# Ivordir/YALPS

Measured on AMD Instinct MI355X. Metric: fp64 pivots/sec on dense m x n tableau, higher is better.
Workload: dtype f64

## Files before the change

### yalps_amd/build.py

```python
import os
import re
import shutil
import subprocess

HERE = os.path.dirname(os.path.abspath(__file__))
ROOT = os.path.dirname(HERE)
LIB = os.path.join(HERE, "libyalps_hip.so")
LIB_STAMPS = os.path.join(HERE, "libyalps_hip_stamps.so")
LINK_LIBS = []
CSRC = os.path.join(HERE, "csrc")
HIP_SRC = os.path.join(CSRC, "yalps_hip.hip")
HIP_UNITS = [HIP_SRC] + [os.path.join(CSRC, f) for f in sorted(os.listdir(CSRC)) if f.startswith("persistent_") and f.endswith(".hip")]
HIP_DEPS = [os.path.join(CSRC, f) for f in sorted(os.listdir(CSRC)) if f.endswith((".cuh", ".inc", ".h")) and not f.startswith(("lp_batch", "lp_dense", "lp_variants", "lp_sens", "lp_warm", "milp_node", "milp_tree", "milp_dense", "wg_queue"))]
LIB_LPBATCH = os.path.join(HERE, "libyalps_lpbatch.so")
LPBATCH_SRC = os.path.join(CSRC, "lp_batch.hip")
QUEUE_DEPS = [os.path.join(CSRC, f) for f in ("wg_queue.cuh", "wg_queue_host.inc", "wg_simplex.cuh", "common.cuh")]
LPBATCH_DEPS = [os.path.join(CSRC, f) for f in ("lp_batch_kernel.cuh", "lp_batch_host.inc", "lp_batch_lib.inc")] + QUEUE_DEPS
LPBATCH_HEADER = os.path.join(ROOT, "include", "yalps_lpbatch.h")
LIB_MILPBATCH = os.path.join(HERE, "libyalps_milpbatch.so")
MILPBATCH_SRC = os.path.join(CSRC, "milp_batch.hip")
MILPBATCH_DEPS = LPBATCH_DEPS + [os.path.join(CSRC, f) for f in ("milp_node_kernel.cuh", "milp_search.inc")] + [LPBATCH_HEADER]
MILPBATCH_HEADER = os.path.join(ROOT, "include", "yalps_milpbatch.h")
LIB_LPVAR = os.path.join(HERE, "libyalps_lpvar.so")
LPVAR_SRC = os.path.join(CSRC, "lp_variants.hip")
LPVAR_DEPS = [os.path.join(CSRC, "lp_variants_kernel.cuh")] + QUEUE_DEPS
LPVAR_HEADER = os.path.join(ROOT, "include", "yalps_lpvar.h")
LIB_LPSENS = os.path.join(HERE, "libyalps_lpsens.so")
LPSENS_SRC = os.path.join(CSRC, "lp_sens.hip")
LPSENS_DEPS = [os.path.join(CSRC, "lp_sens_kernel.cuh")] + LPBATCH_DEPS
LPSENS_HEADER = os.path.join(ROOT, "include", "yalps_lpsens.h")
LIB_LPWARM = os.path.join(HERE, "libyalps_lpwarm.so")
LPWARM_SRC = os.path.join(CSRC, "lp_warm.hip")
LPWARM_DEPS = [os.path.join(CSRC, "lp_warm_kernel.cuh")] + LPBATCH_DEPS + [LPBATCH_HEADER]
LPWARM_HEADER = os.path.join(ROOT, "include", "yalps_lpwarm.h")
LIB_MILPTREE = os.path.join(HERE, "libyalps_milptree.so")
MILPTREE_SRC = os.path.join(CSRC, "milp_tree.hip")
MILPTREE_DEPS = LPBATCH_DEPS + [os.path.join(CSRC, f) for f in ("milp_tree_kernel.cuh", "milp_tree_rules.cuh", "milp_tree_host.inc")] + [LPBATCH_HEADER]
MILPTREE_HEADER = os.path.join(ROOT, "include", "yalps_milptree.h")
LIB_LPDENSE = os.path.join(HERE, "libyalps_lpdense.so")
LPDENSE_SRC = os.path.join(CSRC, "lp_dense.hip")
LPDENSE_DEPS = [os.path.join(CSRC, "lp_dense_kernel.cuh")] + QUEUE_DEPS
LIB_LPDENSE_BOUNDS = os.path.join(HERE, "libyalps_lpdense_bounds.so")
LPDENSE_BOUNDS_SRC = os.path.join(CSRC, "lp_dense_bounds.hip")
LPDENSE_HEADER = os.path.join(ROOT, "include", "yalps_lpdense.h")
LIB_LPDENSE_FREE = os.path.join(HERE, "libyalps_lpdense_free.so")
LPDENSE_FREE_SRC = os.path.join(CSRC, "lp_dense_free.hip")
LIB_MILPDENSE = os.path.join(HERE, "libyalps_milpdense.so")
MILPDENSE_SRC = os.path.join(CSRC, "milp_dense.hip")
MILPDENSE_DEPS = [os.path.join(CSRC, f) for f in ("milp_dense_kernel.cuh", "milp_tree_kernel.cuh", "milp_tree_rules.cuh", "milp_tree_host.inc",
                                                  "lp_batch_kernel.cuh", "milp_dense_bounds_kernel.cuh", "milp_dense_free_kernel.cuh")] + QUEUE_DEPS
MILPDENSE_HEADER = os.path.join(ROOT, "include", "yalps_milpdense.h")
LIB_MILPDENSE_BOUNDS = os.path.join(HERE, "libyalps_milpdense_bounds.so")
MILPDENSE_BOUNDS_SRC = os.path.join(CSRC, "milp_dense_bounds.hip")
MILPDENSE_BOUNDS_DEPS = [os.path.join(CSRC, f) for f in ("milp_dense_bounds_kernel.cuh", "milp_dense_kernel.cuh", "milp_tree_rules.cuh")] + QUEUE_DEPS
LIB_MILPDENSE_FREE = os.path.join(HERE, "libyalps_milpdense_free.so")
MILPDENSE_FREE_SRC = os.path.join(CSRC, "milp_dense_free.hip")
MILPDENSE_FREE_DEPS = [os.path.join(CSRC, "milp_dense_free_kernel.cuh")] + MILPDENSE_BOUNDS_DEPS
OBJ_DIR = os.path.join(HERE, "build")
HEADER = os.path.join(ROOT, "include", "yalps_hip.h")
NAPI_SRC = os.path.join(HERE, "napi", "yalps_napi.cc")
NAPI_OUT = os.path.join(HERE, "napi", "yalps_napi.node")

HIPCC_FLAGS = ["--offload-arch=gfx950", "-O3", "-std=c++17", "-ffp-contract=off", "-fPIC"]


def _stale(out, *srcs):
    return not os.path.exists(out) or any(os.path.getmtime(out) < os.path.getmtime(s) for s in srcs if os.path.exists(s))


def kernel_metadata(lib=LIB):
    import re
    import tempfile
    llvm = "/opt/rocm/lib/llvm/bin"
    with tempfile.TemporaryDirectory() as tmp:
        fat, co = os.path.join(tmp, "fat.bin"), os.path.join(tmp, "dev.co")
        subprocess.run([f"{llvm}/llvm-objcopy", "-O", "binary", "--only-section=.hip_fatbin", lib, fat], check=True)
        magic = b"__CLANG_OFFLOAD_BUNDLE__"
        blob = open(fat, "rb").read()
        starts = [i for i in range(len(blob)) if blob.startswith(magic, i)]
        if not starts:
            raise RuntimeError("no offload bundle in .hip_fatbin of %s" % lib)
        notes = ""
        for k, lo in enumerate(starts):
            part = os.path.join(tmp, "part%d.bin" % k)
            with open(part, "wb") as f:
                f.write(blob[lo:starts[k + 1] if k + 1 < len(starts) else len(blob)])
            subprocess.run([f"{llvm}/clang-offload-bundler", "--unbundle", "--type=o", f"--input={part}",
                            "--targets=hipv4-amdgcn-amd-amdhsa--gfx950", f"--output={co}"], check=True)
            notes += subprocess.run([f"{llvm}/llvm-readelf", "--notes", co], check=True, capture_output=True, text=True).stdout
    kernels, cur = {}, {}
    for line in notes.splitlines():
        m = re.match(r"\s*(?:- )?\.(\w+):\s+(\S+)\s*$", line)
        if not m:
            continue
        key, val = m.groups()
        if key == "agpr_count" and line.lstrip().startswith("- "):
            cur = {}
        cur[key] = val
        if key == "name" and val.startswith("_Z"):
            kernels[val] = cur
    return kernels


NO_SCRATCH = ("lp_sens", "lp_dense", "milp_dense_root_kernel", "milp_dense_solution_kernel", "milp_dense_bounds_root_kernel", "milp_dense_bounds_solution_kernel", "milp_dense_free_root_kernel", "milp_dense_free_solution_kernel", "lp_variants", "lp_warm", "milp_node_kernel", "milp_tree_kernel", "dshard_kernel", "dshard_select_kernel", "dshard_sweep_kernel", "small_kernel", "batch_kernel", "assemble", "resident_kernel", "resident2_kernel", "stream_kernel", "stream2_kernel", "stream3_kernel", "sweep_kernel")


RESIDENT2_SGPR_SPILLS = {(256, 1, 4): 7, (256, 1, 9): 14, (256, 2, 4): 11, (512, 2, 4): 11, (512, 2, 6): 17, (512, 2, 9): 23,
                         (512, 3, 4): 21}


def check_register_budgets(lib=LIB, min_resident=15):
    ks = kernel_metadata(lib)
    resident = {k: v for k, v in ks.items() if "resident_kernel" in k or "resident2_kernel" in k}
    bad = []
    if len(resident) < min_resident:
        bad.append("only %d resident_kernel instantiations in the code object" % len(resident))
    for name, md in sorted(ks.items()):
        if ("resident_kernel" in name or "resident2_kernel" in name) and (int(md["vgpr_count"]) > 256 or int(md["agpr_count"]) != 0):
            bad.append("%s: vgpr_count %s agpr_count %s" % (name, md["vgpr_count"], md["agpr_count"]))
        r2 = re.search(r"resident2_kernelILi(\d+)ELi(\d+)ELi(\d+)EE", name)
        if r2:
            shape = tuple(int(x) for x in r2.groups())
            if shape not in RESIDENT2_SGPR_SPILLS:
                bad.append("%s: no sgpr_spill_count bound for this instantiation" % name)
            elif int(md.get("sgpr_spill_count", 0)) > RESIDENT2_SGPR_SPILLS[shape]:
                bad.append("%s: sgpr_spill_count %s, bound %d" % (name, md.get("sgpr_spill_count"), RESIDENT2_SGPR_SPILLS[shape]))
        if any(tag in name for tag in NO_SCRATCH) and int(md["private_segment_fixed_size"]) != 0:
            bad.append("%s: private_segment_fixed_size %s (scratch)" % (name, md["private_segment_fixed_size"]))
        queue = "lp_dense_free_kernel" in name or "lp_dense_bounds_kernel" in name or "lp_batch_kernel" in name or "milp_node_kernel" in name or "lp_variants_kernel" in name or "lp_sens_kernel" in name or "lp_warm_kernel" in name or "milp_tree_kernel" in name or "lp_dense_kernel" in name or "milp_dense_root_kernel" in name or "milp_dense_bounds_root_kernel" in name or "milp_dense_free_root_kernel" in name
        if queue and int(md["agpr_count"]) != 0:
            bad.append("%s: agpr_count %s" % (name, md["agpr_count"]))
        if queue and int(md["group_segment_fixed_size"]) % 16 != 0:
            bad.append("%s: group_segment_fixed_size %s is not a multiple of 16 (misaligned 128-bit LDS accesses)" % (name, md["group_segment_fixed_size"]))
    if bad and os.environ.get("YALPS_BUILD_ALLOW_SCRATCH") == "1":
        print("register budget violated (YALPS_BUILD_ALLOW_SCRATCH=1: building anyway):\n  " + "\n  ".join(bad))
        return ks
    if bad:
        raise RuntimeError("register budget violated (a spilling variant computes wrong rows):\n  " + "\n  ".join(bad))
    return ks


def build_hip(force=False, verbose=False, stamps=False):
    lib_out = LIB_STAMPS if stamps else LIB
    obj_dir = OBJ_DIR + ("_stamps" if stamps else "")
    if not force and not _stale(lib_out, HEADER, *HIP_UNITS, *HIP_DEPS):
        return lib_out
    hipcc = shutil.which("hipcc") or "/opt/rocm/bin/hipcc"
    os.makedirs(obj_dir, exist_ok=True)
    objs = [os.path.join(obj_dir, os.path.basename(u)[:-4] + ".o") for u in HIP_UNITS]
    flags = HIPCC_FLAGS + (["-DYALPS_STAMPS"] if stamps else [])

    def compile_unit(pair):
        unit, obj = pair
        if not force and not _stale(obj, unit, HEADER, *HIP_DEPS):
            return
        cmd = [hipcc, *flags, "-c", "-o", obj, unit]
        if verbose:
            print(" ".join(cmd), flush=True)
        subprocess.run(cmd, check=True)

    from concurrent.futures import ThreadPoolExecutor
    with ThreadPoolExecutor(max_workers=min(len(objs), os.cpu_count() or 1)) as pool:
        list(pool.map(compile_unit, zip(HIP_UNITS, objs)))
    cmd = [hipcc, "--offload-arch=gfx950", "-shared", "-fPIC", "-o", lib_out + ".tmp", *objs, *LINK_LIBS]
    if verbose:
        print(" ".join(cmd), flush=True)
    subprocess.run(cmd, check=True)
    if not stamps:
        check_register_budgets(lib_out + ".tmp")
    os.replace(lib_out + ".tmp", lib_out)
    return lib_out


def build_single_unit(src, out, deps, header, kernels, force=False, verbose=False, link=()):
    if not force and not _stale(out, header, src, *deps):
        return out
    hipcc = shutil.which("hipcc") or "/opt/rocm/bin/hipcc"
    os.makedirs(OBJ_DIR, exist_ok=True)
    obj = os.path.join(OBJ_DIR, os.path.basename(src)[:-4] + ".o")
    for cmd in ([hipcc, *HIPCC_FLAGS, "-c", "-o", obj, src],
                [hipcc, "--offload-arch=gfx950", "-shared", "-fPIC", "-o", out + ".tmp", obj,
                 *(["-L" + os.path.dirname(out), "-Wl,-rpath,$ORIGIN"] if link else []), *("-l:" + os.path.basename(l) for l in link)]):
        if verbose:
            print(" ".join(cmd), flush=True)
        subprocess.run(cmd, check=True)
    ks = check_register_budgets(out + ".tmp", min_resident=0)
    for kernel in kernels:
        if not any(kernel in k for k in ks):
            raise RuntimeError("no %s in the code object of %s" % (kernel, out))
    os.replace(out + ".tmp", out)
    return out


def build_lpbatch(force=False, verbose=False):
    return build_single_unit(LPBATCH_SRC, LIB_LPBATCH, LPBATCH_DEPS, LPBATCH_HEADER,
                             ("lp_batch_kernel",), force, verbose)


def build_milpbatch(force=False, verbose=False):
    return build_single_unit(MILPBATCH_SRC, LIB_MILPBATCH, MILPBATCH_DEPS, MILPBATCH_HEADER,
                             ("milp_node_kernel", "lp_batch_kernel"), force, verbose)


def build_lpvar(force=False, verbose=False):
    return build_single_unit(LPVAR_SRC, LIB_LPVAR, LPVAR_DEPS, LPVAR_HEADER,
                             ("lp_variants_kernel", "lp_variants_base_kernel"), force, verbose)


def build_lpsens(force=False, verbose=False):
    return build_single_unit(LPSENS_SRC, LIB_LPSENS, LPSENS_DEPS, LPSENS_HEADER,
                             ("lp_sens_kernel",), force, verbose)


def build_lpwarm(force=False, verbose=False):
    return build_single_unit(LPWARM_SRC, LIB_LPWARM, LPWARM_DEPS, LPWARM_HEADER,
                             ("lp_warm_kernel", "lp_warm_image_kernel", "lp_batch_kernel"), force, verbose)


def build_milptree(force=False, verbose=False):
    return build_single_unit(MILPTREE_SRC, LIB_MILPTREE, MILPTREE_DEPS, MILPTREE_HEADER,
                             ("milp_tree_kernel", "lp_batch_kernel"), force, verbose)


def build_lpdense(force=False, verbose=False):
    bounds = build_single_unit(LPDENSE_BOUNDS_SRC, LIB_LPDENSE_BOUNDS, LPDENSE_DEPS, LPDENSE_HEADER,
                               ("lp_dense_bounds_kernel",), force, verbose)
    free = build_single_unit(LPDENSE_FREE_SRC, LIB_LPDENSE_FREE, LPDENSE_DEPS, LPDENSE_HEADER,
                             ("lp_dense_free_kernel",), force, verbose)
    return build_single_unit(LPDENSE_SRC, LIB_LPDENSE, LPDENSE_DEPS + [bounds, free], LPDENSE_HEADER,
                             ("lp_dense_kernel",), force, verbose, link=(bounds, free))


def build_milpdense(force=False, verbose=False):
    bounds = build_milpdense_bounds(force, verbose)
    free = build_milpdense_free(force, verbose)
    return build_single_unit(MILPDENSE_SRC, LIB_MILPDENSE, MILPDENSE_DEPS + [bounds, free], MILPDENSE_HEADER,
                             ("milp_dense_root_kernel", "milp_dense_solution_kernel", "milp_tree_kernel"), force, verbose, link=(bounds, free))


def build_milpdense_bounds(force=False, verbose=False):
    return build_single_unit(MILPDENSE_BOUNDS_SRC, LIB_MILPDENSE_BOUNDS, MILPDENSE_BOUNDS_DEPS, MILPDENSE_HEADER,
                             ("milp_dense_bounds_root_kernel", "milp_dense_bounds_solution_kernel"), force, verbose)


def build_milpdense_free(force=False, verbose=False):
    return build_single_unit(MILPDENSE_FREE_SRC, LIB_MILPDENSE_FREE, MILPDENSE_FREE_DEPS, MILPDENSE_HEADER,
                             ("milp_dense_free_root_kernel", "milp_dense_free_solution_kernel"), force, verbose)


def build_napi(force=False, verbose=False):
    inc = "/usr/include/node"
    if not os.path.exists(os.path.join(inc, "node_api.h")) or not os.path.exists(NAPI_SRC):
        return None
    if not force and not _stale(NAPI_OUT, NAPI_SRC, HEADER):
        return NAPI_OUT
    cmd = ["g++", "-O2", "-std=c++17", "-fPIC", "-shared", "-I", inc, "-I", os.path.join(ROOT, "include"),
           "-o", NAPI_OUT, NAPI_SRC, "-ldl"]
    if verbose:
        print(" ".join(cmd))
    subprocess.run(cmd, check=True)
    return NAPI_OUT


if __name__ == "__main__":
    import sys
    if "stamps" in sys.argv[1:]:
        print(build_hip(verbose=True, stamps=True))
        raise SystemExit(0)
    print(build_hip(force=True, verbose=True))
    print(build_lpbatch(force=True, verbose=True))
    print(build_milpbatch(force=True, verbose=True))
    print(build_lpvar(force=True, verbose=True))
    print(build_lpsens(force=True, verbose=True))
    print(build_lpwarm(force=True, verbose=True))
    print(build_milptree(force=True, verbose=True))
    print(build_lpdense(force=True, verbose=True))
    print(build_milpdense(force=True, verbose=True))
    print(build_napi(force=True, verbose=True))
```

### yalps_amd/csrc/resident2_kernel.cuh

```cuda
#pragma once


__device__ __forceinline__ double min_f64_raw(double a, double b) {
    double r;
    asm("v_min_f64 %0, %1, %2" : "=v"(r) : "v"(a), "v"(b));
    return r;
}
constexpr int DPP_ROW_BCAST15 = 0x142, DPP_ROW_BCAST31 = 0x143;
template <int CTRL, int ROW_MASK>
__device__ __forceinline__ int dpp_i32_rm(int v) {
    return __builtin_amdgcn_update_dpp(v, v, CTRL, ROW_MASK, 0xF, false);
}
template <int CTRL, int ROW_MASK>
__device__ __forceinline__ double dpp_f64_rm(double v) {
    const int lo = dpp_i32_rm<CTRL, ROW_MASK>(__double2loint(v)), hi = dpp_i32_rm<CTRL, ROW_MASK>(__double2hiint(v));
    return __hiloint2double(hi, lo);
}
template <int STEPS>
__device__ __forceinline__ double rowN_min_raw(double v) {
    v = min_f64_raw(v, dpp_f64<DPP_XOR1>(v));
    if constexpr (STEPS >= 2) v = min_f64_raw(v, dpp_f64<DPP_XOR2>(v));
    if constexpr (STEPS >= 3) v = min_f64_raw(v, dpp_f64<DPP_HALF_MIRROR>(v));
    if constexpr (STEPS >= 4) v = min_f64_raw(v, dpp_f64<DPP_MIRROR>(v));
    return v;
}
template <int STEPS>
__device__ __forceinline__ int rowN_min(int v) {
    v = min(v, dpp_i32<DPP_XOR1>(v));
    if constexpr (STEPS >= 2) v = min(v, dpp_i32<DPP_XOR2>(v));
    if constexpr (STEPS >= 3) v = min(v, dpp_i32<DPP_HALF_MIRROR>(v));
    if constexpr (STEPS >= 4) v = min(v, dpp_i32<DPP_MIRROR>(v));
    return v;
}
__device__ __forceinline__ KI wave_argmin2(KI v) {
    double m = rowN_min_raw<4>(v.k);
    m = min_f64_raw(m, dpp_f64_rm<DPP_ROW_BCAST15, 0xA>(m));
    m = min_f64_raw(m, dpp_f64_rm<DPP_ROW_BCAST31, 0xC>(m));
    KI r;
    r.k = lane_f64(m, 63);
    const bool hit = v.k == r.k;
    const unsigned long long mask = __builtin_amdgcn_ballot_w64(hit);
    if (__popcll(mask) == 1) {
        r.i = __builtin_amdgcn_readlane(v.i, __ffsll((long long)mask) - 1);
    } else {
        int i = rowN_min<4>(hit ? v.i : INT_MAX);
        i = min(i, dpp_i32_rm<DPP_ROW_BCAST15, 0xA>(i));
        i = min(i, dpp_i32_rm<DPP_ROW_BCAST31, 0xC>(i));
        r.i = __builtin_amdgcn_readlane(i, 63);
    }
    return r;
}
template <int T>
__device__ __forceinline__ KI block_argmin2(KI v, double (*sk)[16], int (*si)[16], int slot) {
    constexpr int NW = T / 64, STEPS = NW == 16 ? 4 : NW == 8 ? 3 : NW == 4 ? 2 : 1;
    static_assert(NW == 2 || NW == 4 || NW == 8 || NW == 16, "waves per workgroup");
    v = wave_argmin2(v);
    const int lane = threadIdx.x & 63, wv = threadIdx.x >> 6;
    if (lane == 0) {
        sk[slot][wv] = v.k;
        si[slot][wv] = v.i;
    }
    __syncthreads();
    const double k = sk[slot][lane & (NW - 1)];
    const int i = si[slot][lane & (NW - 1)];
    const double km = rowN_min_raw<STEPS>(k);
    KI r;
    r.k = uniform_f64(km);
    r.i = __builtin_amdgcn_readfirstlane(rowN_min<STEPS>(k == km ? i : INT_MAX));
    return r;
}

template <int R>
struct Slots {
    static constexpr int W = R <= 4 ? 4 : 8;
    static_assert(R <= W + 1, "row slots per workgroup");
    typedef double V __attribute__((ext_vector_type(W)));
    V v;
    double odd;
    __device__ __forceinline__ double at(int g) const { return g < W ? v[g & (W - 1)] : odd; }
    __device__ __forceinline__ void set(int g, double a) {
        if (g < W)
            v[g & (W - 1)] = a;
        else
            odd = a;
    }
    __device__ __forceinline__ static int vslot(int s) {
        s = __builtin_amdgcn_readfirstlane(s);
        if constexpr (R > W) return s < W ? s : 0;
        return s;
    }
    __device__ __forceinline__ double get(int s) const {
        const double a = v[vslot(s)];
        if constexpr (R > W) return s < W ? a : odd;
        return a;
    }
    __device__ __forceinline__ void put(int s, double a) {
        if constexpr (R > W) {
            const int i = vslot(s);
            const double keep = v[i];
            v[i] = s < W ? a : keep;
            odd = s < W ? odd : a;
        } else {
            v[vslot(s)] = a;
        }
    }
};

template <int R, int N>
struct SlotRows {
    Slots<R> head;
    SlotRows<R, N - 1> tail;
    template <int K>
    __device__ __forceinline__ Slots<R> &el() {
        if constexpr (K == 0)
            return head;
        else
            return tail.template el<K - 1>();
    }
};
template <int R>
struct SlotRows<R, 0> {};
template <int K>
struct IntC {
    static constexpr int value = K;
};
template <int N, int K = 0, class F>
__device__ __forceinline__ void static_for(F &&f) {
    if constexpr (K < N) {
        f(IntC<K>{});
        static_for<N, K + 1>(f);
    }
}
#define EACH_ELEM(k, j, e, xe)                                                                                          \
    static_for<2 * J>([&](auto k) __attribute__((always_inline)) {                                                     \
        constexpr int j = decltype(k)::value / 2, e = decltype(k)::value % 2;                                         \
        [[maybe_unused]] Slots<R> &xe = x.template el<decltype(k)::value>();
#define END_EACH_ELEM });
#define KEEP_ARM(k) asm volatile("" ::"i"(decltype(k)::value))

template <int T, int J, int R>
__global__ __launch_bounds__(T) void resident2_kernel(Desc d, int parity, int chunk) {
    constexpr int SPLIT = YALPS_SPLIT_NUM * R / 4;
    constexpr unsigned FULL = (1u << (2 * J)) - 1u;
    __shared__ double sk[2][16];
    __shared__ int si[2][16];
    __shared__ double sh_cf[2][R + 2];
    __shared__ double sh_nq[R + 2];
    __shared__ double sh_raw[R + 2];
    __shared__ double sh_ck;
    __shared__ int sh_ci, sh_cg, sh_fail, sh_flag, sh_verdict, sh_pnz;
    extern __shared__ int sh_perm[];

    const int NB = d.nb, b = blockIdx.x;
    int tid = threadIdx.x;
#define FRESH_TID() asm volatile("" : "+v"(tid))
    const int wave = __builtin_amdgcn_readfirstlane(tid >> 6);
    const YState *Sin = d.st + parity;
    YState *Sout = d.st + (parity ^ 1);
    const YConst *C = d.cst;
    if (Sin->status != RUNNING) {
        if (b == 0 && tid == 0) state_copy(Sout, Sin);
        return;
    }
    const int h = C->height, n = d.n, pitch = d.pitch, w = d.w;
    const double precision = C->precision, max_pivots = C->max_pivots;
    const int mbuf = Sin->mbuf;
    const double *matA = d.mat[mbuf];
    const double *rhsA = d.rhs[mbuf];
    int phase = Sin->phase;
    double iter = Sin->iter;
    int64_t pivots = Sin->pivots;
    int64_t hist_len = Sin->hist_len;
    const bool check_cycles = C->check_cycles != 0;
    asm volatile("" : "+v"(iter));
    asm volatile("" : "+v"(pivots));
    int slot = 0;

    int cofs[J];
#pragma unroll
    for (int j = 0; j < J; j++) {
        const int c0 = 2 * (tid + j * T);
        cofs[j] = c0 < pitch ? c0 : 0;
    }
    unsigned padmask = 0;
#pragma unroll
    for (int j = 0; j < J; j++)
#pragma unroll
        for (int k = 0; k < 2; k++)
            if (2 * (tid + j * T) + k >= n) padmask |= 1u << (2 * j + k);
    SlotRows<R, 2 * J> x;
    double2 o[J];
    EACH_ELEM(k, j, e, xe)
        xe.v = 0.0;
        xe.odd = 0.0;
    END_EACH_ELEM
#pragma unroll
    for (int j = 0; j < J; j++) {
        o[j] = *reinterpret_cast<const double2 *>(matA + cofs[j]);
        if (padmask & (1u << (2 * j))) o[j].x = -INFINITY;
        if (padmask & (1u << (2 * j + 1))) o[j].y = -INFINITY;
    }
#pragma unroll
    for (int g = 0; g < R; g++) {
        const int r = b + NB * g;
        const double *mr = matA + (size_t)(r < h ? r : b) * pitch;
        double2 t[J];
#pragma unroll
        for (int j = 0; j < J; j++) t[j] = *reinterpret_cast<const double2 *>(mr + cofs[j]);
        EACH_ELEM(k, j, e, xe)
            xe.set(g, e ? t[j].y : t[j].x);
        END_EACH_ELEM
    }
    const int nlive = b < h ? (h - b + NB - 1) / NB : 0;
    auto my_row = [&]() __attribute__((always_inline)) { return b + NB * tid; };
    auto my_live = [&]() __attribute__((always_inline)) { return tid < R && tid < nlive; };
    double my_rhs = rhsA[my_live() ? my_row() : 0];
    if (b == 0) {
        for (int i = tid; i < d.perm_len; i += T) {
            sh_perm[i] = d.var[i];
            sh_perm[d.perm_len + i] = d.pos[i];
        }
    }
    if (tid == 0) sh_fail = 0;
    __syncthreads();

    int la = 0;
    double la_val = 0.0;
    unsigned epoch = 0;
    int cur = 0;
    auto price = [&]() __attribute__((always_inline)) {
        double best = precision;
        int bi = INT_MAX;
#pragma unroll
        for (int j = 0; j < J; j++) {
            const int c0 = 2 * (tid + j * T);
            if (o[j].x > best) {
                best = o[j].x;
                bi = c0 + 1;
            }
            if (o[j].y > best) {
                best = o[j].y;
                bi = c0 + 2;
            }
        }
        KI v = {bi == INT_MAX ? INFINITY : -best, bi};
        v = block_argmin2<T>(v, sk, si, slot);
        slot ^= 1;
        la = v.i == INT_MAX ? 0 : v.i;
        la_val = -v.k;
    };
    auto deposit_la = [&](const double2 (&pvn)[J], unsigned nzmask, bool pending) __attribute__((always_inline)) {
        const int ula = (la - 1) >> 1, ela = (la - 1) & 1, lt = ula % T, lj = ula / T;
        if (la > 0 && wave == (lt >> 6)) {
            if (tid == lt) {
                EACH_ELEM(k, j, e, xe)
                    if (j == lj && e == ela) {
#pragma unroll
                        for (int g = 0; g < R; g++) sh_raw[g] = xe.at(g);
                        KEEP_ARM(k);
                    }
                END_EACH_ELEM
                if (pending) {
#pragma unroll
                    for (int j = 0; j < J; j++)
                        if (j == lj) {
                            sh_raw[R] = elem(pvn[j], ela);
                            sh_pnz = (nzmask >> (2 * j + ela)) & 1u;
                        }
                }
            }
        }
        __syncthreads();
    };
    auto candidate = [&](int kind, double value, int which, bool barrier) __attribute__((always_inline)) {
        if (wave == 0) {
            KI c = {INFINITY, INT_MAX};
            const int my_r = my_row();
            if (my_live() && my_r >= 1) {
                if (kind == 1) {
                    if (my_rhs < -precision) {
                        c.k = my_rhs;
                        c.i = my_r;
                    }
                } else if (la > 0 && value > precision) {
                    const double ratio = my_rhs / value;
                    if (ratio < INFINITY) {
                        c.k = (ratio <= precision) ? -INFINITY : ratio;
                        c.i = my_r;
                    }
                }
            }
            if (kind == 2 && tid < R) sh_cf[which][tid] = value;
            c = wave_argmin2(c);
            if (tid == 0) {
                sh_ck = c.k;
                sh_ci = c.i;
                sh_cg = c.i == INT_MAX ? 0 : c.i / NB;
            }
        }
        if (barrier) __syncthreads();
    };
    auto publish_flag = [&]() __attribute__((always_inline)) {
        const int par = epoch & 1;
        asm volatile("s_waitcnt vmcnt(0)" ::: "memory");
        __syncthreads();
        if (tid == 0)
            st16_sc1(reinterpret_cast<double *>(d.rc_flag[par] + 2 * b),
                     make_double2(sh_ck, __longlong_as_double((long long)(((unsigned long long)epoch << 32) | (unsigned)sh_ci))));
    };
    auto publish_stores = [&](int cg) __attribute__((always_inline)) {
        epoch++;
        double *dst = d.rc_rows[epoch & 1] + (size_t)b * pitch;
        double2 crow[J];
        EACH_ELEM(k, j, e, xe)
            if (e)
                crow[j].y = xe.get(cg);
            else
                crow[j].x = xe.get(cg);
        END_EACH_ELEM
#pragma unroll
        for (int j = 0; j < J; j++) {
            const int c0 = 2 * (tid + j * T);
            if (c0 < pitch) st16_sc1(dst + c0, crow[j]);
        }
        if (tid == cg) st_sc1(d.rc_key[epoch & 1] + b, my_rhs);
    };
    int done = 0, term = RUNNING;
    double term_result = NAN;
    bool stop = false;
#ifdef YALPS_STAMPS
    unsigned long long st_acc[20] = {}, st_last = 0, st_t0 = 0, st_r0 = 0;
#endif
    auto check = [&]() __attribute__((always_inline)) {
        if (done == chunk) {
            stop = true;
        } else if (__builtin_amdgcn_ballot_w64(!(iter < max_pivots)) != 0) {
            term = YALPS_CYCLED;
            stop = true;
        } else if (phase == 2 && la == 0) {
            term = YALPS_OPTIMAL;
            stop = true;
        }
    };
    const double2 no_row[J] = {};
    auto open_round = [&]() __attribute__((always_inline)) {
        double value = 0.0;
        if (phase == 2) {
            deposit_la(no_row, 0u, false);
            if (tid < R) value = sh_raw[tid];
        }
        candidate(phase, value, cur, true);
        publish_stores(__builtin_amdgcn_readfirstlane(sh_cg));
        publish_flag();
    };

    price();
    check();
    if (!stop) open_round();
#ifdef YALPS_STAMPS
    asm volatile("s_memtime %0\n\ts_memrealtime %1\n\ts_waitcnt lgkmcnt(0)" : "=s"(st_t0), "=s"(st_r0)::"memory");
    st_last = st_t0;
#endif
    while (!stop) {
        FRESH_TID();
        const int par = epoch & 1;
        KI c = {INFINITY, INT_MAX};
        if (tid < NB) {
            unsigned long long f = 0;
            unsigned spins = 0;
            [[maybe_unused]] unsigned long long spin_t0 = 0;
            double2 rec;
            for (;;) {
                rec = ld16_sc1_one(d.rc_flag[par] + 2 * tid);
                f = (unsigned long long)__double_as_longlong(rec.y);
                if ((unsigned)(f >> 32) == epoch) break;
                if (RESIDENT_SPIN_EXPIRED(spins, spin_t0, d.rc_err)) {
                    sh_fail = 1;
                    __hip_atomic_store(d.rc_err, 1, __ATOMIC_RELAXED, __HIP_MEMORY_SCOPE_AGENT);
                    break;
                }
                __builtin_amdgcn_s_sleep(2);
            }
            c.i = (int)(unsigned)f;
            c.k = rec.x;
#ifdef YALPS_AB_POLL_GUARD
            if (c.i != INT_MAX && (unsigned)c.i >= (unsigned)h) {
                sh_fail = 1;
                __hip_atomic_store(d.rc_err, 1, __ATOMIC_RELAXED, __HIP_MEMORY_SCOPE_AGENT);
            }
#endif
        }
        YSTAMP(0);
        c = block_argmin2<T>(c, sk, si, slot);
        slot ^= 1;
        YSTAMP(1);
        if (sh_fail) return;
        if (c.i == INT_MAX) {
            if (phase == 1) {
                phase = 2;
                iter = 0.0;
                hist_len = 0;
                check();
                if (!stop) open_round();
            } else {
                term = YALPS_UNBOUNDED;
                term_result = (double)la;
                stop = true;
            }
            YSTAMP(14);
            continue;
        }
#if defined(YALPS_AB_RETURN_GUARD) || defined(YALPS_AB_NOGUARD) || defined(YALPS_AB_POLL_GUARD)
        const int row = c.i, owner = row % NB;
#else
        const int row_in = c.i, row = (unsigned)row_in < (unsigned)h ? row_in : 0, owner = row % NB;
        if (row != row_in && tid == 0) __hip_atomic_store(d.rc_err, 1, __ATOMIC_RELAXED, __HIP_MEMORY_SCOPE_AGENT);
#endif
#ifdef YALPS_AB_RETURN_GUARD
        if ((unsigned)row >= (unsigned)h) {
            if (tid == 0) __hip_atomic_store(d.rc_err, 1, __ATOMIC_RELAXED, __HIP_MEMORY_SCOPE_AGENT);
            return;
        }
#endif
        const double *src = d.rc_rows[par] + (size_t)owner * pitch;
        double2 pv[J];
        const double rhs_row = ld_sc1(d.rc_key[par] + owner);
        double q = ld_sc1(src + (phase == 2 ? la - 1 : 0));
        ld16_sc1<J>(pv, src, cofs);
        YSTAMP(2);
        int col = la;
        double coef0 = la_val;
        if (phase == 1) {
            KI e = {INFINITY, INT_MAX};
#pragma unroll
            for (int j = 0; j < J; j++) {
                const int c0 = 2 * (tid + j * T);
#pragma unroll
                for (int k = 0; k < 2; k++) {
                    const double coefficient = elem(pv[j], k);
                    if (c0 + k < n && coefficient < -precision) {
                        const double ratio = -elem(o[j], k) / coefficient;
                        if (ratio > -INFINITY && ki_better(-ratio, c0 + k + 1, e.k, e.i)) {
                            e.k = -ratio;
                            e.i = c0 + k + 1;
                        }
                    }
                }
            }
            e = block_argmin2<T>(e, sk, si, slot);
            slot ^= 1;
            if (e.i == INT_MAX) {
                term = YALPS_INFEASIBLE;
                stop = true;
                continue;
            }
            col = e.i;
            const int ucol1 = (col - 1) >> 1, ecol1 = (col - 1) & 1;
            if (tid == ucol1 % T) {
                EACH_ELEM(k, j, e, xe)
                    if (j == ucol1 / T && e == ecol1) {
#pragma unroll
                        for (int g = 0; g < R; g++) sh_cf[cur][g] = xe.at(g);
                        KEEP_ARM(k);
                    }
                END_EACH_ELEM
#pragma unroll
                for (int j = 0; j < J; j++)
                    if (j == ucol1 / T) {
                        sh_cf[cur][R] = elem(o[j], ecol1);
                        sh_cf[cur][R + 1] = elem(pv[j], ecol1);
                    }
            }
            __syncthreads();
            coef0 = sh_cf[cur][R];
            q = sh_cf[cur][R + 1];
        }
        if (check_cycles) {
            int cycled = 0;
            if (b == 0) {
                const int leaving = sh_perm[w + row], entering = sh_perm[col];
                cycled = has_cycle(C, hist_len, leaving, entering, &sh_flag) ? 1 : 0;
                if (tid == 0)
                    __hip_atomic_store(d.rc_verdict + par, ((unsigned long long)epoch << 32) | (unsigned)cycled,
                                       __ATOMIC_RELAXED, __HIP_MEMORY_SCOPE_AGENT);
            } else {
                if (tid == 0) {
                    unsigned long long v = 0;
                    unsigned spins = 0;
                    [[maybe_unused]] unsigned long long spin_t0 = 0;
                    for (;;) {
                        v = __hip_atomic_load(d.rc_verdict + par, __ATOMIC_RELAXED, __HIP_MEMORY_SCOPE_AGENT);
                        if ((unsigned)(v >> 32) == epoch) break;
                        if (RESIDENT_SPIN_EXPIRED(spins, spin_t0, d.rc_err)) {
                            sh_fail = 1;
                            __hip_atomic_store(d.rc_err, 1, __ATOMIC_RELAXED, __HIP_MEMORY_SCOPE_AGENT);
                            break;
                        }
                        __builtin_amdgcn_s_sleep(2);
                    }
                    sh_verdict = (int)(unsigned)v;
                }
                __syncthreads();
                if (sh_fail) return;
                cycled = sh_verdict;
            }
            hist_len += 1;
            if (cycled) {
                term = YALPS_CYCLED;
                stop = true;
                continue;
            }
        }
        YSTAMP(3);
        FRESH_TID();
        const int ucol = (col - 1) >> 1, ecol = (col - 1) & 1, col_tid = ucol % T, col_j = ucol / T;
        const int col_wave = col_tid >> 6;
        Slots<R> cf;
        cf.v = 0.0;
        cf.odd = 0.0;
#pragma unroll
        for (int g = 0; g < R; g++) cf.set(g, sh_cf[cur][g]);
        const double my_coef = tid < R ? sh_cf[cur][tid] : 0.0;
        const int lane = tid & 63;
        const double lane_cf = sh_cf[cur][lane < R ? lane : 0];
        const unsigned touched = (unsigned)__builtin_amdgcn_ballot_w64(lane < R && lane < nlive && fabs(lane_cf) > 1e-16);
        const bool all_touched = touched == (1u << (nlive < R ? nlive : R)) - 1u;
        unsigned nzmask = 0;
#pragma unroll
        for (int j = 0; j < J; j++) {
            const bool nzx = fabs(pv[j].x) > 1e-16, nzy = fabs(pv[j].y) > 1e-16;
            pv[j].x = nzx ? pv[j].x / q : 0.0;
            pv[j].y = nzy ? pv[j].y / q : 0.0;
            nzmask |= (nzx ? 1u : 0u) << (2 * j) | (nzy ? 1u : 0u) << (2 * j + 1);
        }
        const bool fast = __builtin_amdgcn_ballot_w64(((nzmask | padmask) & FULL) != FULL) == 0;
        const bool nz_rhs = fabs(rhs_row) > 1e-16;
        const int lslot = owner == b ? row / NB : -1;
        double my_nq = 0.0;
        if (wave == 0) {
            const double num = tid < R ? -my_coef : tid == R + 1 ? 1.0 : rhs_row;
            const double quot = num / q;
            my_nq = quot;
            if (tid < R || tid == R + 1) sh_nq[tid] = quot;
            const double rhs_q = lane_f64(quot, R + 2);
            if (my_live()) {
                const double pn_rhs = nz_rhs ? rhs_q : 0.0;
                if (tid == lslot)
                    my_rhs = pn_rhs;
                else if (fabs(my_coef) > 1e-16 && nz_rhs) {
                    const double prod = my_coef * pn_rhs;
                    my_rhs = my_rhs - prod;
                }
            }
        }
        if (fabs(coef0) > 1e-16) {
            if (fast) {
#pragma unroll
                for (int j = 0; j < J; j++) {
                    const double px = coef0 * pv[j].x, py = coef0 * pv[j].y;
                    o[j].x = o[j].x - px;
                    o[j].y = o[j].y - py;
                }
            } else {
#pragma unroll
                for (int j = 0; j < J; j++) {
                    const double px = coef0 * pv[j].x, py = coef0 * pv[j].y;
                    const double nx = o[j].x - px, ny = o[j].y - py;
                    o[j].x = (nzmask & (1u << (2 * j))) ? nx : o[j].x;
                    o[j].y = (nzmask & (1u << (2 * j + 1))) ? ny : o[j].y;
                }
            }
            if (wave == col_wave) {
                if (tid == col_tid) {
                    const double nq0 = -coef0 / q;
#pragma unroll
                    for (int j = 0; j < J; j++)
                        if (j == col_j) {
                            if (ecol)
                                o[j].y = nq0;
                            else
                                o[j].x = nq0;
                        }
                }
            }
        }
        YSTAMP(5);
        iter += 1.0;
        pivots += 1;
        done += 1;
        price();
        check();
        YSTAMP(6);
        FRESH_TID();
        auto finish_rows = [&](unsigned set) __attribute__((always_inline)) {
            const unsigned pivbit = lslot >= 0 ? (1u << lslot) & set : 0u;
            const unsigned elim = set & touched & ~pivbit;
            const bool holds_col = wave == col_wave && tid == col_tid;
            if constexpr (R <= 4) {
                double2 r[R][J];
                EACH_ELEM(k, j, e, xe)
#pragma unroll
                    for (int g = 0; g < R; g++) {
                        if (e)
                            r[g][j].y = xe.at(g);
                        else
                            r[g][j].x = xe.at(g);
                    }
                END_EACH_ELEM
#pragma unroll
                for (int g = 0; g < R; g++) {
                    if ((pivbit >> g) & 1u) {
#pragma unroll
                        for (int j = 0; j < J; j++) r[g][j] = pv[j];
                    } else if ((elim >> g) & 1u) {
                        if (fast) {
#pragma unroll
                            for (int j = 0; j < J; j++) {
                                const double px = cf.at(g) * pv[j].x, py = cf.at(g) * pv[j].y;
                                r[g][j].x = r[g][j].x - px;
                                r[g][j].y = r[g][j].y - py;
                            }
                        } else {
#pragma unroll
                            for (int j = 0; j < J; j++) {
                                const double px = cf.at(g) * pv[j].x, py = cf.at(g) * pv[j].y;
                                const double nx = r[g][j].x - px, ny = r[g][j].y - py;
                                r[g][j].x = (nzmask & (1u << (2 * j))) ? nx : r[g][j].x;
                                r[g][j].y = (nzmask & (1u << (2 * j + 1))) ? ny : r[g][j].y;
                            }
                        }
                    }
                }
                if (wave == col_wave && (elim | pivbit) != 0) {
                    if (tid == col_tid) {
#pragma unroll
                        for (int g = 0; g < R; g++) {
                            if (((elim | pivbit) >> g) & 1u) {
                                const double v = sh_nq[((pivbit >> g) & 1u) ? R + 1 : g];
#pragma unroll
                                for (int j = 0; j < J; j++)
                                    if (j == col_j) {
                                        if (ecol)
                                            r[g][j].y = v;
                                        else
                                            r[g][j].x = v;
                                    }
                            }
                        }
                    }
                }
                EACH_ELEM(k, j, e, xe)
#pragma unroll
                    for (int g = 0; g < R; g++) xe.set(g, e ? r[g][j].y : r[g][j].x);
                END_EACH_ELEM
            } else {
                if (pivbit) {
                    const double inv = sh_nq[R + 1];
                    EACH_ELEM(k, j, e, xe)
                        const double p = e ? pv[j].y : pv[j].x;
                        xe.put(lslot, (holds_col && j == col_j && e == ecol) ? inv : p);
                    END_EACH_ELEM
                }
#pragma clang loop unroll(disable)
                for (unsigned m = elim; m != 0; m &= m - 1) {
                    const int g = __builtin_ctz(m);
                    const double c = cf.get(g), nq = sh_nq[g];
                    EACH_ELEM(k, j, e, xe)
                        const double old = xe.get(g);
                        const double p = c * (e ? pv[j].y : pv[j].x);
                        double nv = old - p;
                        if (!fast) nv = (nzmask & (1u << (2 * j + e))) ? nv : old;
                        xe.put(g, (holds_col && j == col_j && e == ecol) ? nq : nv);
                    END_EACH_ELEM
                }
            }
        };
        constexpr unsigned ONE = 1, ALL = (ONE << R) - 1, LOW = (ONE << SPLIT) - 1;
        if (!stop) {
            double value = 0.0;
            if (phase == 2) {
                deposit_la(pv, nzmask, true);
                YSTAMP(7);
                if (tid < R) {
                    value = sh_raw[tid];
                    if (tid == lslot)
                        value = la == col ? sh_nq[R + 1] : sh_raw[R];
                    else if (my_live() && fabs(my_coef) > 1e-16) {
                        if (la == col)
                            value = my_nq;
                        else if (sh_pnz) {
                            const double prod = my_coef * sh_raw[R];
                            value = value - prod;
                        }
                    }
                }
            }
            if (fast && all_touched) {
                candidate(phase, value, cur ^ 1, true);
                const int cg = __builtin_amdgcn_readfirstlane(sh_cg);
                double2 cand[J];
                const double ccf = cf.get(cg);
                EACH_ELEM(k, j, e, xe)
                    if (e)
                        cand[j].y = xe.get(cg);
                    else
                        cand[j].x = xe.get(cg);
                END_EACH_ELEM
                if (cg == lslot) {
#pragma unroll
                    for (int j = 0; j < J; j++) cand[j] = pv[j];
                } else {
#pragma unroll
                    for (int j = 0; j < J; j++) {
                        const double px = ccf * pv[j].x, py = ccf * pv[j].y;
                        cand[j].x = cand[j].x - px;
                        cand[j].y = cand[j].y - py;
                    }
                }
                if (wave == col_wave) {
                    if (tid == col_tid) {
                        const double v = sh_nq[cg == lslot ? R + 1 : cg];
#pragma unroll
                        for (int j = 0; j < J; j++)
                            if (j == col_j) {
                                if (ecol)
                                    cand[j].y = v;
                                else
                                    cand[j].x = v;
                            }
                    }
                }
                epoch++;
                {
                    double *dst = d.rc_rows[epoch & 1] + (size_t)b * pitch;
#pragma unroll
                    for (int j = 0; j < J; j++) {
                        const int c0 = 2 * (tid + j * T);
                        if (c0 < pitch) st16_sc1(dst + c0, cand[j]);
                    }
                    if (tid == cg) st_sc1(d.rc_key[epoch & 1] + b, my_rhs);
                }
                publish_flag();
                EACH_ELEM(k, j, e, xe)
                    const double p = e ? pv[j].y : pv[j].x;
#pragma unroll
                    for (int g = 0; g < R; g++) {
                        const double prod = cf.at(g) * p;
                        xe.set(g, xe.at(g) - prod);
                    }
                    if (lslot >= 0) xe.put(lslot, p);
                END_EACH_ELEM
                if (wave == col_wave) {
                    const bool holds_col = tid == col_tid;
                    int nl = nlive;
                    asm volatile("" : "+s"(nl));
                    EACH_ELEM(k, j, e, xe)
                        if (j == col_j && e == ecol) {
#pragma unroll
                            for (int g = 0; g < R; g++)
                                if (g < nl) {
                                    const double v = sh_nq[g == lslot ? R + 1 : g];
                                    xe.set(g, holds_col ? v : xe.at(g));
                                }
                            KEEP_ARM(k);
                        }
                    END_EACH_ELEM
                }
            } else {
                candidate(phase, value, cur ^ 1, true);
                YSTAMP(8);
                const int cg = __builtin_amdgcn_readfirstlane(sh_cg);
                finish_rows(ONE << cg);
                YSTAMP(9);
                publish_stores(cg);
                YSTAMP(10);
                if constexpr (SPLIT > 0) finish_rows(LOW & ~(ONE << cg));
                YSTAMP(11);
                publish_flag();
                YSTAMP(12);
                finish_rows(ALL & ~LOW & ~(ONE << cg));
            }
        } else {
            finish_rows(ALL);
        }
        cur ^= 1;
        if (b == 0 && tid == 0) {
            int *var = sh_perm, *pos = sh_perm + d.perm_len;
            const int leaving = var[w + row], entering = var[col];
            var[w + row] = entering;
            var[col] = leaving;
            pos[leaving] = col;
            pos[entering] = w + row;
        }
        YSTAMP(13);
    }
#ifdef YALPS_STAMPS
    if (tid == 0 && d.dbg) {
        unsigned long long t1, r1;
        asm volatile("s_memtime %0\n\ts_memrealtime %1\n\ts_waitcnt lgkmcnt(0)" : "=s"(t1), "=s"(r1)::"memory");
        unsigned long long *out = d.dbg + (size_t)b * STAMP_WORDS;
#pragma unroll
        for (int k = 0; k < 20; k++) out[k] += st_acc[k];
        out[20] += (unsigned long long)done;
        out[21] += t1 - st_t0;
        out[22] += r1 - st_r0;
    }
#endif

    double *matB = d.mat[mbuf ^ 1];
    double *rhsB = d.rhs[mbuf ^ 1];
    int nl = nlive;
    asm volatile("" : "+s"(nl));
#pragma unroll
    for (int g = 0; g < R; g++) {
        const int r = b + NB * g;
        if (g < nl) {
            double *mr = matB + (size_t)r * pitch;
            double2 t[J];
            EACH_ELEM(k, j, e, xe)
                if (e)
                    t[j].y = xe.at(g);
                else
                    t[j].x = xe.at(g);
            END_EACH_ELEM
#pragma unroll
            for (int j = 0; j < J; j++) {
                const int c0 = 2 * (tid + j * T);
                if (c0 < pitch) *reinterpret_cast<double2 *>(mr + c0) = t[j];
            }
        }
    }
    if (my_live()) rhsB[my_row()] = my_rhs;
    if (b == 0) {
        __syncthreads();
        for (int i = tid; i < d.perm_len; i += T) {
            d.var[i] = sh_perm[i];
            d.pos[i] = sh_perm[d.perm_len + i];
        }
        if (tid == 0) {
            if (term == YALPS_OPTIMAL) term_result = round_to_precision(my_rhs, precision);
            Sout->status = term;
            Sout->phase = phase;
            Sout->bootstrap = 1;
            Sout->la = 0;
            Sout->pbuf = 0;
            Sout->mbuf = mbuf ^ 1;
            Sout->pause = 0;
            Sout->dec_valid = 0;
            Sout->dec_row = 0;
            Sout->dec_col = 0;
            Sout->swap_valid = 0;
            Sout->swap_row = 0;
            Sout->swap_col = 0;
            Sout->pad_ = 0;
            Sout->hist_len = hist_len;
            Sout->iter = iter;
            Sout->result = term_result;
            Sout->pivots = pivots;
        }
    }
}
#undef EACH_ELEM
#undef FRESH_TID
#undef KEEP_ARM
#undef END_EACH_ELEM
```

Measured before the change: 195,000.

## Fuse ratio-test deposit into candidate via cross-lane writelane, dropping LDS barrier

Merges the deposit_la and candidate steps. The owning wave now moves the entering column's slot values into lanes with v_writelane and readlane instead of staging them through shared memory (sh_raw, sh_pnz). This removes one __syncthreads and an LDS round trip per pivot, and the ratio test runs directly in that wave. A new sh_rhs shared array carries the per-slot rhs values, and the SGPR spill bounds are retuned, so register pressure and scalar spills may shift.

```diff
diff --git a/yalps_amd/build.py b/yalps_amd/build.py
--- a/yalps_amd/build.py
+++ b/yalps_amd/build.py
@@ -105,8 +105,8 @@
 NO_SCRATCH = ("lp_sens", "lp_dense", "milp_dense_root_kernel", "milp_dense_solution_kernel", "milp_dense_bounds_root_kernel", "milp_dense_bounds_solution_kernel", "milp_dense_free_root_kernel", "milp_dense_free_solution_kernel", "lp_variants", "lp_warm", "milp_node_kernel", "milp_tree_kernel", "dshard_kernel", "dshard_select_kernel", "dshard_sweep_kernel", "small_kernel", "batch_kernel", "assemble", "resident_kernel", "resident2_kernel", "stream_kernel", "stream2_kernel", "stream3_kernel", "sweep_kernel")
 
 
-RESIDENT2_SGPR_SPILLS = {(256, 1, 4): 7, (256, 1, 9): 14, (256, 2, 4): 11, (512, 2, 4): 11, (512, 2, 6): 17, (512, 2, 9): 23,
-                         (512, 3, 4): 21}
+RESIDENT2_SGPR_SPILLS = {(256, 1, 4): 6, (256, 1, 9): 8, (256, 2, 4): 12, (512, 2, 4): 12, (512, 2, 6): 14, (512, 2, 9): 18,
+                         (512, 3, 4): 19}
 
 
 def check_register_budgets(lib=LIB, min_resident=15):
diff --git a/yalps_amd/csrc/resident2_kernel.cuh b/yalps_amd/csrc/resident2_kernel.cuh
--- a/yalps_amd/csrc/resident2_kernel.cuh
+++ b/yalps_amd/csrc/resident2_kernel.cuh
@@ -50,6 +50,13 @@
     }
     return r;
 }
+template <int LANE>
+__device__ __forceinline__ double to_lane_f64(double old, double s) {
+    int hi = __double2hiint(old), lo = __double2loint(old);
+    asm("v_writelane_b32 %0, %1, %2" : "+v"(hi) : "s"(__double2hiint(s)), "n"(LANE));
+    asm("v_writelane_b32 %0, %1, %2" : "+v"(lo) : "s"(__double2loint(s)), "n"(LANE));
+    return __hiloint2double(hi, lo);
+}
 template <int T>
 __device__ __forceinline__ KI block_argmin2(KI v, double (*sk)[16], int (*si)[16], int slot) {
     constexpr int NW = T / 64, STEPS = NW == 16 ? 4 : NW == 8 ? 3 : NW == 4 ? 2 : 1;
@@ -106,6 +113,13 @@
     }
 };
 
+template <int R, int G = 0>
+__device__ __forceinline__ double slots_to_lanes(const Slots<R> &xe, int src, double acc = 0.0) {
+    if constexpr (G < R)
+        return slots_to_lanes<R, G + 1>(xe, src, to_lane_f64<G>(acc, lane_f64(xe.at(G), src)));
+    else
+        return acc;
+}
 template <int R, int N>
 struct SlotRows {
     Slots<R> head;
@@ -146,9 +160,9 @@
     __shared__ int si[2][16];
     __shared__ double sh_cf[2][R + 2];
     __shared__ double sh_nq[R + 2];
-    __shared__ double sh_raw[R + 2];
+    __shared__ double sh_rhs[R];
     __shared__ double sh_ck;
-    __shared__ int sh_ci, sh_cg, sh_fail, sh_flag, sh_verdict, sh_pnz;
+    __shared__ int sh_ci, sh_cg, sh_fail, sh_flag, sh_verdict;
     extern __shared__ int sh_perm[];
 
     const int NB = d.nb, b = blockIdx.x;
@@ -222,6 +236,7 @@
         }
     }
     if (tid == 0) sh_fail = 0;
+    if (tid < R) sh_rhs[tid] = my_rhs;
     __syncthreads();
 
     int la = 0;
@@ -249,56 +264,74 @@
         la = v.i == INT_MAX ? 0 : v.i;
         la_val = -v.k;
     };
-    auto deposit_la = [&](const double2 (&pvn)[J], unsigned nzmask, bool pending) __attribute__((always_inline)) {
-        const int ula = (la - 1) >> 1, ela = (la - 1) & 1, lt = ula % T, lj = ula / T;
-        if (la > 0 && wave == (lt >> 6)) {
-            if (tid == lt) {
+    auto candidate = [&](const double2 (&pvn)[J], unsigned nzmask, bool pending, int lslot, int col, int which) __attribute__((always_inline)) {
+        const int lane = tid & 63;
+        if (phase == 1) {
+            if (wave == 0) {
+                KI c = {INFINITY, INT_MAX};
+                const int my_r = my_row();
+                if (my_live() && my_r >= 1 && my_rhs < -precision) {
+                    c.k = my_rhs;
+                    c.i = my_r;
+                }
+                c = wave_argmin2(c);
+                if (tid == 0) {
+                    sh_ck = c.k;
+                    sh_ci = c.i;
+                    sh_cg = c.i == INT_MAX ? 0 : c.i / NB;
+                }
+            }
+        } else {
+            const int ula = (la - 1) >> 1, ela = (la - 1) & 1, lt = ula % T, lj = ula / T;
+            if (la > 0 && wave == (lt >> 6)) {
+                const int src = lt & 63;
+                const int ls = lane < R ? lane : 0;
+                double my_coef = sh_cf[cur][ls], my_nq = sh_nq[ls], inv_q = sh_nq[R + 1], rhs_g = sh_rhs[ls];
+                double value = 0.0;
                 EACH_ELEM(k, j, e, xe)
                     if (j == lj && e == ela) {
-#pragma unroll
-                        for (int g = 0; g < R; g++) sh_raw[g] = xe.at(g);
+                        value = slots_to_lanes<R>(xe, src);
                         KEEP_ARM(k);
                     }
                 END_EACH_ELEM
+                asm volatile("" : "+v"(my_coef), "+v"(my_nq), "+v"(inv_q), "+v"(rhs_g));
                 if (pending) {
+                    double pn = 0.0;
 #pragma unroll
                     for (int j = 0; j < J; j++)
-                        if (j == lj) {
-                            sh_raw[R] = elem(pvn[j], ela);
-                            sh_pnz = (nzmask >> (2 * j + ela)) & 1u;
+                        if (j == lj) pn = lane_f64(ela ? pvn[j].y : pvn[j].x, src);
+                    const bool pnz = ((unsigned)__builtin_amdgcn_readlane((int)nzmask, src) >> (2 * lj + ela)) & 1u;
+                    if (lane < R) {
+                        if (lane == lslot)
+                            value = la == col ? inv_q : pn;
+                        else if (lane < nlive && fabs(my_coef) > 1e-16) {
+                            if (la == col)
+                                value = my_nq;
+                            else if (pnz) {
+                                const double prod = my_coef * pn;
+                                value = value - prod;
+                            }
                         }
-                }
-            }
-        }
-        __syncthreads();
-    };
-    auto candidate = [&](int kind, double value, int which, bool barrier) __attribute__((always_inline)) {
-        if (wave == 0) {
-            KI c = {INFINITY, INT_MAX};
-            const int my_r = my_row();
-            if (my_live() && my_r >= 1) {
-                if (kind == 1) {
-                    if (my_rhs < -precision) {
-                        c.k = my_rhs;
-                        c.i = my_r;
-                    }
-                } else if (la > 0 && value > precision) {
-                    const double ratio = my_rhs / value;
+                    }
+                }
+                KI c = {INFINITY, INT_MAX};
+                if (lane < R && lane < nlive && b + NB * lane >= 1 && value > precision) {
+                    const double ratio = rhs_g / value;
                     if (ratio < INFINITY) {
                         c.k = (ratio <= precision) ? -INFINITY : ratio;
-                        c.i = my_r;
-                    }
-                }
-            }
-            if (kind == 2 && tid < R) sh_cf[which][tid] = value;
-            c = wave_argmin2(c);
-            if (tid == 0) {
-                sh_ck = c.k;
-                sh_ci = c.i;
-                sh_cg = c.i == INT_MAX ? 0 : c.i / NB;
-            }
-        }
-        if (barrier) __syncthreads();
+                        c.i = lane;
+                    }
+                }
+                if (lane < R) sh_cf[which][lane] = value;
+                c = wave_argmin2(c);
+                if (lane == 0) {
+                    sh_ck = c.k;
+                    sh_ci = c.i == INT_MAX ? INT_MAX : b + NB * c.i;
+                    sh_cg = c.i == INT_MAX ? 0 : c.i;
+                }
+            }
+        }
+        __syncthreads();
     };
     auto publish_flag = [&]() __attribute__((always_inline)) {
         const int par = epoch & 1;
@@ -344,12 +377,7 @@
     };
     const double2 no_row[J] = {};
     auto open_round = [&]() __attribute__((always_inline)) {
-        double value = 0.0;
-        if (phase == 2) {
-            deposit_la(no_row, 0u, false);
-            if (tid < R) value = sh_raw[tid];
-        }
-        candidate(phase, value, cur, true);
+        candidate(no_row, 0u, false, -1, 0, cur);
         publish_stores(__builtin_amdgcn_readfirstlane(sh_cg));
         publish_flag();
     };
@@ -536,11 +564,9 @@
         const bool fast = __builtin_amdgcn_ballot_w64(((nzmask | padmask) & FULL) != FULL) == 0;
         const bool nz_rhs = fabs(rhs_row) > 1e-16;
         const int lslot = owner == b ? row / NB : -1;
-        double my_nq = 0.0;
         if (wave == 0) {
             const double num = tid < R ? -my_coef : tid == R + 1 ? 1.0 : rhs_row;
             const double quot = num / q;
-            my_nq = quot;
             if (tid < R || tid == R + 1) sh_nq[tid] = quot;
             const double rhs_q = lane_f64(quot, R + 2);
             if (my_live()) {
@@ -552,6 +578,7 @@
                     my_rhs = my_rhs - prod;
                 }
             }
+            if (tid < R) sh_rhs[tid] = my_rhs;
         }
         if (fabs(coef0) > 1e-16) {
             if (fast) {
@@ -677,27 +704,11 @@
         };
         constexpr unsigned ONE = 1, ALL = (ONE << R) - 1, LOW = (ONE << SPLIT) - 1;
         if (!stop) {
-            double value = 0.0;
-            if (phase == 2) {
-                deposit_la(pv, nzmask, true);
-                YSTAMP(7);
-                if (tid < R) {
-                    value = sh_raw[tid];
-                    if (tid == lslot)
-                        value = la == col ? sh_nq[R + 1] : sh_raw[R];
-                    else if (my_live() && fabs(my_coef) > 1e-16) {
-                        if (la == col)
-                            value = my_nq;
-                        else if (sh_pnz) {
-                            const double prod = my_coef * sh_raw[R];
-                            value = value - prod;
-                        }
-                    }
-                }
-            }
+            candidate(pv, nzmask, true, lslot, col, cur ^ 1);
+            YSTAMP(7);
+            const int cg = __builtin_amdgcn_readfirstlane(sh_cg);
+            YSTAMP(8);
             if (fast && all_touched) {
-                candidate(phase, value, cur ^ 1, true);
-                const int cg = __builtin_amdgcn_readfirstlane(sh_cg);
                 double2 cand[J];
                 const double ccf = cf.get(cg);
                 EACH_ELEM(k, j, e, xe)
@@ -730,6 +741,7 @@
                             }
                     }
                 }
+                YSTAMP(9);
                 epoch++;
                 {
                     double *dst = d.rc_rows[epoch & 1] + (size_t)b * pitch;
@@ -740,7 +752,9 @@
                     }
                     if (tid == cg) st_sc1(d.rc_key[epoch & 1] + b, my_rhs);
                 }
+                YSTAMP(10);
                 publish_flag();
+                YSTAMP(12);
                 EACH_ELEM(k, j, e, xe)
                     const double p = e ? pv[j].y : pv[j].x;
 #pragma unroll
@@ -767,9 +781,6 @@
                     END_EACH_ELEM
                 }
             } else {
-                candidate(phase, value, cur ^ 1, true);
-                YSTAMP(8);
-                const int cg = __builtin_amdgcn_readfirstlane(sh_cg);
                 finish_rows(ONE << cg);
                 YSTAMP(9);
                 publish_stores(cg);
```

After: 198,600, median of 6. No clear change (+1.9%).
